# CVMI-Lab/DODA

Hardware: AMD Instinct MI355X
Metric: active-voxels/sec fwd+bwd SparseConv U-Net, ScanNet 2cm (higher is better)
Workload: dtype bf16; 1 GPU; cfgs/scannet SparseConv U-Net training step (voxel pooling + fwd + CE + bwd + SGD), 2 cm voxels, 4 scenes/GPU x ~150000 active voxels, random-init weights; global_batch=4, voxels_per_gpu=601279, points_per_gpu=781042, parallelism=dp1, n_classes=20, grad_sync=deferred multi-layer wgrad + bucketed all-reduce, collectives=none (single process), prefetch_gate=off, grad_exchange=no process group

## Files before the change

doda_amd/csrc/spconv_wgrad.hip:

```cpp
#include "wgrad_pairs.hpp"
#include <stdlib.h>
#include <string.h>
#include <mutex>
#include <vector>

typedef float f32x4 __attribute__((ext_vector_type(4)));
typedef short s16x4 __attribute__((ext_vector_type(4)));
typedef __bf16 bf16x8 __attribute__((ext_vector_type(8)));
typedef unsigned int u32x4 __attribute__((ext_vector_type(4)));

namespace {

constexpr int RT = 64;
constexpr int MAX_OGW = 7;
constexpr int PAD = 8;

struct F32 {
    typedef float elem;
    typedef f32x4 frag;
    typedef f32x4 vec;
    static constexpr int VEC = 4;
    static constexpr int KSTEPS = RT / 4;
    typedef float kfrag;
    template <int STRIDE>
    static __device__ __forceinline__ void frags(const elem *tile, int g, int i, int col0, kfrag (&out)[KSTEPS]) {
#pragma unroll
        for (int ks = 0; ks < KSTEPS; ++ks) out[ks] = tile[(ks * 4 + g) * STRIDE + col0 + i];
    }
    static __device__ __forceinline__ f32x4 mma(kfrag a, kfrag b, f32x4 c) {
        return __builtin_amdgcn_mfma_f32_16x16x4f32(a, b, c, 0, 0, 0);
    }
};

struct F32S : F32 {
    static constexpr int KSTEPS = RT / 16;
    struct kfrag { unsigned hi[2], lo[2]; };
    template <int STRIDE>
    static __device__ __forceinline__ void frags(const elem *tile, int g, int i, int col0, kfrag (&out)[KSTEPS]) {
        typedef __bf16 bf16x2 __attribute__((ext_vector_type(2)));
        typedef float f32x2 __attribute__((ext_vector_type(2)));
#pragma unroll
        for (int ks = 0; ks < KSTEPS; ++ks) {
            float v[4];
#pragma unroll
            for (int q = 0; q < 4; ++q) v[q] = tile[(ks * 16 + 4 * g + q) * STRIDE + col0 + i];
#pragma unroll
            for (int h = 0; h < 2; ++h) {
                const f32x2 a = {v[2 * h], v[2 * h + 1]};
                const unsigned hu = __builtin_bit_cast(unsigned, __builtin_convertvector(a, bf16x2));
                const f32x2 res = {a[0] - __uint_as_float(hu << 16), a[1] - __uint_as_float(hu & 0xffff0000u)};
                out[ks].hi[h] = hu;
                out[ks].lo[h] = __builtin_bit_cast(unsigned, __builtin_convertvector(res, bf16x2));
            }
        }
    }
    static __device__ __forceinline__ f32x4 mma(const kfrag &a, const kfrag &b, f32x4 c) {
        const u32x4 av = {a.hi[0], a.hi[1], a.lo[0], a.lo[1]};
        const u32x4 b1 = {b.hi[0], b.hi[1], b.hi[0], b.hi[1]}, b2 = {b.lo[0], b.lo[1], b.lo[0], b.lo[1]};
        c = __builtin_amdgcn_mfma_f32_16x16x32_bf16(__builtin_bit_cast(bf16x8, av), __builtin_bit_cast(bf16x8, b1), c, 0, 0, 0);
        return __builtin_amdgcn_mfma_f32_16x16x32_bf16(__builtin_bit_cast(bf16x8, av), __builtin_bit_cast(bf16x8, b2), c, 0, 0, 0);
    }
};

struct BF16 {
    typedef unsigned short elem;
    typedef s16x4 frag;
    typedef u32x4 vec;
    static constexpr int VEC = 8;
    static constexpr int KSTEPS = RT / 32;
    typedef bf16x8 kfrag;
    template <int STRIDE>
    static __device__ __forceinline__ void frags(const elem *tile, int g, int i, int col0, kfrag (&out)[KSTEPS]) {
        static_assert(KSTEPS == 2, "two k-steps of 32 rows");
        const unsigned addr = (unsigned)(uintptr_t)(tile + (8 * g + (i >> 2)) * STRIDE + col0 + 4 * (i & 3));
        s16x4 lo0, hi0, lo1, hi1;
        asm volatile("ds_read_b64_tr_b16 %0, %4\n\t"
                     "ds_read_b64_tr_b16 %1, %4 offset:%5\n\t"
                     "ds_read_b64_tr_b16 %2, %4 offset:%6\n\t"
                     "ds_read_b64_tr_b16 %3, %4 offset:%7\n\t"
                     "s_waitcnt lgkmcnt(0)"
                     : "=&v"(lo0), "=&v"(hi0), "=&v"(lo1), "=&v"(hi1)
                     : "v"(addr), "n"(4 * STRIDE * 2), "n"(32 * STRIDE * 2), "n"(36 * STRIDE * 2)
                     : "memory");
        typedef short s16x8 __attribute__((ext_vector_type(8)));
        const s16x8 k0 = __builtin_shufflevector(lo0, hi0, 0, 1, 2, 3, 4, 5, 6, 7);
        const s16x8 k1 = __builtin_shufflevector(lo1, hi1, 0, 1, 2, 3, 4, 5, 6, 7);
        out[0] = __builtin_bit_cast(bf16x8, k0);
        out[1] = __builtin_bit_cast(bf16x8, k1);
    }
    static __device__ __forceinline__ f32x4 mma(kfrag a, kfrag b, f32x4 c) {
        return __builtin_amdgcn_mfma_f32_16x16x32_bf16(a, b, c, 0, 0, 0);
    }
};

template <class T, int TA, int TB, int OGW, bool VOK>
__device__ __forceinline__ void wgrad_body(const typename T::elem *__restrict__ a, int ca,
                                           const typename T::elem *__restrict__ b, int cb,
                                           const int32_t *__restrict__ tbl, int ld, int K,
                                           int n_rows, int rows_per_chunk, int n_tag,
                                           int n_tbg, int n_og, float *__restrict__ partial, int item) {
    typedef typename T::elem elem;
    typedef typename T::frag frag;
    typedef typename T::kfrag kfrag;
    constexpr int SA = TA * 16 + PAD, SB = TB * 16 + PAD;
    __shared__ __attribute__((aligned(16))) elem b_tile[RT * SB];
    __shared__ __attribute__((aligned(16))) elem a_tile[4][RT * SA];

    const int lane = threadIdx.x & 63, wid = threadIdx.x >> 6;
    const int i = lane & 15, g = lane >> 4;
    const int n_grp = n_tag * n_tbg * n_og;
    const int chunk = item / n_grp;
    int grp = item % n_grp;
    const int tag = grp % n_tag; grp /= n_tag;
    const int tbg = grp % n_tbg;
    const int o_base = (grp / n_tbg) * (4 * OGW);
    const int ca0 = tag * TA * 16, cb0 = tbg * TB * 16;

    f32x4 acc[OGW][TA][TB];
#pragma unroll
    for (int oo = 0; oo < OGW; ++oo)
#pragma unroll
        for (int x_ = 0; x_ < TA; ++x_)
#pragma unroll
            for (int y_ = 0; y_ < TB; ++y_) acc[oo][x_][y_] = (f32x4){0.f, 0.f, 0.f, 0.f};

    const long long r_begin = (long long)chunk * rows_per_chunk;
    long long r_end = r_begin + rows_per_chunk;
    if (r_end > n_rows) r_end = n_rows;

    elem *my_a = a_tile[wid];

    typedef typename T::vec vec;
    constexpr int VEC = T::VEC, NVA = TA * 16 / VEC, NVB = TB * 16 / VEC;
    auto load_vec = [&](const elem *p, const elem *safe, int c, int cmax, bool ok) -> vec {
        const bool live = ok && c < cmax;
        if constexpr (VOK) {
            return *reinterpret_cast<const vec *>(live ? p : safe);
        } else {
            vec v = vec{};
            if (live) {
                elem tmp[VEC];
#pragma unroll
                for (int q = 0; q < VEC; ++q) tmp[q] = (c + q < cmax) ? p[q] : (elem)0;
                v = *reinterpret_cast<const vec *>(tmp);
            }
            return v;
        }
    };
    auto gather_row = [&](int idx, vec (&dst)[NVA]) {
#pragma unroll
        for (int f = 0; f < NVA; ++f) {
            const int c = ca0 + f * VEC;
            dst[f] = load_vec(a + (long long)(idx >= 0 ? idx : 0) * ca + c, a, c, ca, idx >= 0);
        }
    };

    constexpr int NDY = (RT * NVB + 255) / 256;
    vec dy_reg[NDY];
    int idx_n[OGW];
    auto load_dy = [&](long long r0) {
#pragma unroll
        for (int k = 0; k < NDY; ++k) {
            const int e = threadIdx.x + k * 256;
            const int r = e / NVB, f = e - r * NVB;
            const long long row = r0 + r;
            const int c = cb0 + f * VEC;
            dy_reg[k] = load_vec(b + (row < r_end ? row : 0) * cb + c, b, c, cb, e < RT * NVB && row < r_end);
        }
    };
    auto load_idx = [&](long long r0) {
#pragma unroll
        for (int oo = 0; oo < OGW; ++oo) {
            const int o = o_base + wid + 4 * oo;
            const long long row = r0 + lane;
            idx_n[oo] = tbl[(o < K && row < r_end) ? (long long)o * ld + row : 0];
        }
    };

    vec rows_cur[NVA], rows_nxt[NVA];
    if (r_begin < r_end) {
        load_dy(r_begin);
        load_idx(r_begin);
        gather_row((o_base + wid < K && r_begin + lane < r_end) ? idx_n[0] : -1, rows_cur);
    }
    for (long long r0 = r_begin; r0 < r_end; r0 += RT) {
        doda_sync();
#pragma unroll
        for (int k = 0; k < NDY; ++k) {
            const int e = threadIdx.x + k * 256;
            if (e < RT * NVB) {
                const int r = e / NVB, f = e - r * NVB;
                const bool live = r0 + r < r_end && cb0 + f * VEC < cb;
                *reinterpret_cast<vec *>(&b_tile[r * SB + f * VEC]) = (VOK && !live) ? vec{} : dy_reg[k];
            }
        }
        int idx[OGW];
#pragma unroll
        for (int oo = 0; oo < OGW; ++oo)
            idx[oo] = (o_base + wid + 4 * oo < K && r0 + lane < r_end) ? idx_n[oo] : -1;
        const bool more = r0 + RT < r_end;
        if (more) {
            load_dy(r0 + RT);
            load_idx(r0 + RT);
        }
        doda_sync();
        kfrag bf[TB][T::KSTEPS];
#pragma unroll
        for (int y_ = 0; y_ < TB; ++y_) T::template frags<SB>(b_tile, g, i, y_ * 16, bf[y_]);

#pragma unroll
        for (int oo = 0; oo < OGW; ++oo) {
            if (oo + 1 < OGW) gather_row(idx[oo + 1], rows_nxt);
            else if (more) gather_row((o_base + wid < K && r0 + RT + lane < r_end) ? idx_n[0] : -1, rows_nxt);
            if (__ballot(idx[oo] >= 0) != 0ull) {
#pragma unroll
                for (int f = 0; f < NVA; ++f) {
                    const bool live = idx[oo] >= 0 && ca0 + f * VEC < ca;
                    *reinterpret_cast<vec *>(&my_a[lane * SA + f * VEC]) = (VOK && !live) ? vec{} : rows_cur[f];
                }
                __builtin_amdgcn_wave_barrier();
#pragma unroll
                for (int x_ = 0; x_ < TA; ++x_) {
                    kfrag af[T::KSTEPS];
                    T::template frags<SA>(my_a, g, i, x_ * 16, af);
#pragma unroll
                    for (int ks = 0; ks < T::KSTEPS; ++ks)
#pragma unroll
                        for (int y_ = 0; y_ < TB; ++y_)
                            acc[oo][x_][y_] = T::mma(af[ks], bf[y_][ks], acc[oo][x_][y_]);
                }
                __builtin_amdgcn_wave_barrier();
            }
#pragma unroll
            for (int f = 0; f < NVA; ++f) rows_cur[f] = rows_nxt[f];
        }
    }

    float *out = partial + (long long)chunk * K * ca * cb;
#pragma unroll
    for (int oo = 0; oo < OGW; ++oo) {
        const int o = o_base + wid + 4 * oo;
        if (o < K) {
#pragma unroll
            for (int x_ = 0; x_ < TA; ++x_)
#pragma unroll
                for (int y_ = 0; y_ < TB; ++y_)
#pragma unroll
                    for (int r = 0; r < 4; ++r) {
                        const int ci = ca0 + x_ * 16 + 4 * g + r, co = cb0 + y_ * 16 + i;
                        if (ci < ca && co < cb)
                            out[((long long)o * ca + ci) * cb + co] = acc[oo][x_][y_][r];
                    }
        }
    }
}

struct WJob {
    const void *a, *b;
    const int32_t *tbl;
    float *out;
    int ca, cb, ld, K, n_rows, rows_per_chunk, n_tag, n_tbg, n_og, blk_end;
};
struct RJob {
    const float4 *partial;
    float4 *dw;
    long long n_quad;
    int R, blk_end, accumulate, pad;
};

template <class J>
__device__ __forceinline__ int find_job(const J *jobs, int n_jobs, int blk) {
    int lo = 0, hi = n_jobs - 1;
    while (lo < hi) {
        const int mid = (lo + hi) >> 1;
        if (blk < jobs[mid].blk_end) hi = mid; else lo = mid + 1;
    }
    return lo;
}

template <class T, int TA, int TB, int OGW, bool VOK>
__global__ __launch_bounds__(256) void wgrad_multi_kernel(const WJob *__restrict__ jobs, int n_jobs) {
    const int j = find_job(jobs, n_jobs, (int)blockIdx.x);
    const WJob d = jobs[j];
    const int first = j == 0 ? 0 : jobs[j - 1].blk_end;
    wgrad_body<T, TA, TB, OGW, VOK>((const typename T::elem *)d.a, d.ca, (const typename T::elem *)d.b, d.cb,
                                    d.tbl, d.ld, d.K, d.n_rows, d.rows_per_chunk, d.n_tag, d.n_tbg, d.n_og,
                                    d.out, (int)blockIdx.x - first);
}

__global__ __launch_bounds__(256) void wgrad_reduce_multi(const RJob *__restrict__ jobs, int n_jobs) {
    __shared__ float4 part[256];
    const int j = find_job(jobs, n_jobs, (int)blockIdx.x);
    const RJob d = jobs[j];
    const int first = j == 0 ? 0 : jobs[j - 1].blk_end;
    const int RL = d.pad, EL = 256 / RL;
    const int el = (int)threadIdx.x % EL, rl = (int)threadIdx.x / EL;
    const long long q = (long long)((int)blockIdx.x - first) * EL + el;
    float4 s = make_float4(0.f, 0.f, 0.f, 0.f);
    if (q < d.n_quad)
        for (int r = rl; r < d.R; r += RL) {
            const float4 v = d.partial[(long long)r * d.n_quad + q];
            s.x += v.x; s.y += v.y; s.z += v.z; s.w += v.w;
        }
    part[rl * EL + el] = s;
    doda_sync();
    if (rl == 0 && q < d.n_quad) {
        float4 t = part[el];
        for (int r = 1; r < RL; ++r) {
            const float4 v = part[r * EL + el];
            t.x += v.x; t.y += v.y; t.z += v.z; t.w += v.w;
        }
        if (d.accumulate) {
            const float4 old = d.dw[q];
            t.x += old.x; t.y += old.y; t.z += old.z; t.w += old.w;
        }
        d.dw[q] = t;
    }
}

__global__ __launch_bounds__(256) void wgrad_reduce(const float *__restrict__ partial, int R,
                                                    long long n_elem, float *__restrict__ dw,
                                                    int accumulate = 0) {
    __shared__ float part[16][17];
    const int el = threadIdx.x & 15, rl = threadIdx.x >> 4;
    const long long e = (long long)blockIdx.x * 16 + el;
    float s = 0.f;
    if (e < n_elem)
        for (int r = rl; r < R; r += 16) s += partial[(long long)r * n_elem + e];
    part[rl][el] = s;
    doda_sync();
    if (rl == 0 && e < n_elem) {
        float t = 0.f;
#pragma unroll
        for (int r = 0; r < 16; ++r) t += part[r][el];
        dw[e] = accumulate ? dw[e] + t : t;
    }
}


struct Plan {
    int TA, TB, OGW, n_og, n_tag, n_tbg, R, rows_per_chunk;
};
static const int MULTI_MIN_ROWS = getenv("DODA_WGRAD_MIN_ROWS") ? atoi(getenv("DODA_WGRAD_MIN_ROWS")) : 512;

Plan make_plan(int K, int ca, int cb, int n_rows, int elem_bytes, bool multi = false) {
    Plan p;
    const int ta = (ca + 15) / 16, tb = (cb + 15) / 16;
    p.TA = (ta % 2 == 0) ? 2 : 1;
    p.TB = (tb % 2 == 0) ? 2 : 1;
    static const bool no33 = getenv("DODA_WGRAD_NO33") && getenv("DODA_WGRAD_NO33")[0] == '1';
    if (ta == 3 && tb == 3 && elem_bytes == 2 && K > 8 && !no33) { p.TA = 3; p.TB = 3; }
    p.n_tag = ta / p.TA;
    p.n_tbg = tb / p.TB;
    p.OGW = (p.TA * p.TB == 4 || elem_bytes == 2) ? 4 : MAX_OGW;
    if (p.TA * p.TB == 9) p.OGW = 2;
    if (K <= 8) p.OGW = (p.TA * p.TB == 4) ? 2 : 2;
    p.n_og = div_up(K, 4 * p.OGW);
    const int gy = p.n_tag * p.n_tbg * p.n_og;
    const int rows = n_rows > 0 ? n_rows : 1;
    static const int t33 = getenv("DODA_WGRAD_T33") ? atoi(getenv("DODA_WGRAD_T33")) : 128;
    const int target = p.TA * p.TB == 9 ? t33 : (multi ? 512 : ((p.TA * p.TB == 4) ? 512 : 1024));
    int R = div_up(target, gy);
    const int max_r = multi ? (rows / MULTI_MIN_ROWS > 1 ? rows / MULTI_MIN_ROWS : 1) : div_up(rows, RT);
    if (R > max_r) R = max_r;
    if (R < 1) R = 1;
    p.rows_per_chunk = div_up(div_up(rows, R), RT) * RT;
    p.R = div_up(rows, p.rows_per_chunk);
    (void)K;
    return p;
}

struct JobPlan {
    Plan p;
    int esz, vok, key;
    int split;
    size_t ws_off;
    long long n_elem;
};

bool plan_job(const doda_wgrad_job &j, JobPlan *out) {
    if (j.ca <= 0 || j.cb <= 0 || j.K <= 0 || j.K > 4 * MAX_OGW || j.n_rows <= 0 || j.ld < j.n_rows || !j.a ||
        !j.b || !j.tbl || !j.dw || (j.elem_bytes != 2 && j.elem_bytes != 4))
        return false;
    out->esz = j.elem_bytes;
    out->vok = ((size_t)j.ca * j.elem_bytes % 16 == 0) && ((size_t)j.cb * j.elem_bytes % 16 == 0) &&
               ((uintptr_t)j.a % 16 == 0) && ((uintptr_t)j.b % 16 == 0);
    out->p = make_plan(j.K, j.ca, j.cb, j.n_rows, j.elem_bytes, true);
    {
        static const long long min_rows = [] { const char *e = getenv("DODA_F32_WGRAD_SPLIT_ROWS"); return e && *e ? atoll(e) : -1ll; }();
        out->split = (j.elem_bytes == 4 && min_rows >= 0 && (long long)j.n_rows >= min_rows) ? 1 : 0;
    }
    out->key = ((((j.elem_bytes * 4 + out->p.TA) * 4 + out->p.TB) * 8 + out->p.OGW) * 2 + out->vok) * 2 + out->split;
    out->n_elem = (long long)j.K * j.ca * j.cb;
    return true;
}

template <class T>
void launch_multi_variant(const Plan &p, int vok, int total_blocks, const WJob *jobs_dev, int n, hipStream_t s) {
    const dim3 grid(total_blocks), block(256);
#define GO(TA, TB, OG)                                                                             \
    do {                                                                                           \
        if (vok) hipLaunchKernelGGL((wgrad_multi_kernel<T, TA, TB, OG, true>), grid, block, 0, s, jobs_dev, n); \
        else hipLaunchKernelGGL((wgrad_multi_kernel<T, TA, TB, OG, false>), grid, block, 0, s, jobs_dev, n); \
    } while (0)
    if (p.OGW == 2) {
        if (p.TA == 3 && p.TB == 3) GO(3, 3, 2);
        else if (p.TA == 1 && p.TB == 1) GO(1, 1, 2);
        else if (p.TA == 2 && p.TB == 1) GO(2, 1, 2);
        else if (p.TA == 1 && p.TB == 2) GO(1, 2, 2);
        else GO(2, 2, 2);
    } else if (p.OGW == 4 && p.TA == 1 && p.TB == 1) GO(1, 1, 4);
    else if (p.OGW == 4 && p.TA == 2 && p.TB == 1) GO(2, 1, 4);
    else if (p.OGW == 4 && p.TA == 1 && p.TB == 2) GO(1, 2, 4);
    else if (p.TA == 1 && p.TB == 1) GO(1, 1, 7);
    else if (p.TA == 2 && p.TB == 1) GO(2, 1, 7);
    else if (p.TA == 1 && p.TB == 2) GO(1, 2, 7);
    else GO(2, 2, 4);
#undef GO
}

struct Staging {
    std::mutex mu;
    void *host = nullptr;
    size_t cap = 0;
    hipEvent_t ev = nullptr;
    int ev_dev = -1;
    bool pending = false;
};
Staging g_staging;
}

enum { J_SKIP = 0, J_ZERO = 1, J_DENSE = 2, J_PAIRS = 3, J_TILE = 4, J_WIDE = 5 };

static int wdma_min_rows() {
    static const int v = getenv("DODA_WDMA_MIN_ROWS") ? atoi(getenv("DODA_WDMA_MIN_ROWS")) : 32768;
    return v;
}

static int classify(const doda_wgrad_job &j) {
    if (j.n_rows == 0 && j.dw && j.K > 0 && j.ca > 0 && j.cb > 0)
        return (j.flags & DODA_WGRAD_ACCUMULATE) ? J_SKIP : J_ZERO;
    if (doda_wwide::eligible(j) && !doda_pairs::eligible(j)) return J_WIDE;
    if (j.tilebook && j.tbl && j.elem_bytes == 2 && j.ca % 16 == 0 && j.ca <= 64 && j.cb % 16 == 0 && j.cb <= 64 &&
        j.K == 27 && j.n_rows > 0 && j.a && j.b && j.dw &&
        j.n_a == j.n_rows && j.ld >= j.n_rows && (size_t)j.n_rows * 128 < 0x7ffffff0ull && (size_t)j.K * j.ld * 4 < 0xffffffffull &&
        !(((uintptr_t)j.a | (uintptr_t)j.b | (uintptr_t)j.tilebook) & 15) && doda_wdma::enabled() &&
        (j.n_rows >= wdma_min_rows() || !doda_pairs::eligible(j)))
        return J_TILE;
    static const bool no_pairs = getenv("DODA_WGRAD_NO_PAIRS") && getenv("DODA_WGRAD_NO_PAIRS")[0] == '1';
    if (doda_pairs::eligible(j) && (!no_pairs || !j.tbl)) return J_PAIRS;
    return J_DENSE;
}

static std::vector<int> wide_chunks(const doda_wgrad_job *jobs_h, const std::vector<int> &idx) {
    std::vector<int> rpc;
    for (int k : idx) rpc.push_back(make_plan(jobs_h[k].K, jobs_h[k].ca, jobs_h[k].cb, jobs_h[k].n_rows, 2, true).rows_per_chunk);
    return rpc;
}

static size_t tile_blocks(const doda_wgrad_job &j) { return (size_t)(j.ca / 16) * (j.cb / 16); }

static bool dense_needs_partial(const JobPlan &jp, const doda_wgrad_job &j) {
    return jp.p.R > 1 || (j.flags & DODA_WGRAD_ACCUMULATE);
}

extern "C" size_t doda_spconv_wgrad_multi_workspace_bytes(const doda_wgrad_job *jobs_h, int32_t n_jobs) {
    if (!jobs_h || n_jobs <= 0) return 0;
    size_t total = 0;
    std::vector<int> wide_jobs;
    for (int k = 0; k < n_jobs; ++k) {
        const int cls = classify(jobs_h[k]);
        if (cls == J_WIDE) { wide_jobs.push_back(k); continue; }
        if (cls == J_PAIRS) { total += doda_pairs::partial_bytes(jobs_h[k]); continue; }
        if (cls == J_TILE) { total += tile_blocks(jobs_h[k]) * align_up(doda_wdma::partial_bytes(jobs_h[k].n_rows), 256); continue; }
        if (cls != J_DENSE) continue;
        JobPlan jp;
        if (!plan_job(jobs_h[k], &jp)) continue;
        if (dense_needs_partial(jp, jobs_h[k])) total += align_up((size_t)jp.p.R * jp.n_elem * 4, 256);
    }
    const std::vector<int> rpc = wide_chunks(jobs_h, wide_jobs);
    total += doda_wwide::partial_bytes(jobs_h, wide_jobs.data(), rpc.data(), (int)wide_jobs.size());
    return total < 256 ? 256 : total;
}

extern "C" size_t doda_spconv_wgrad_multi_desc_bytes(int32_t n_jobs) {
    size_t per = sizeof(WJob) + sizeof(RJob) > doda_pairs::desc_bytes_per_job()
                     ? sizeof(WJob) + sizeof(RJob) : doda_pairs::desc_bytes_per_job();
    if (per < doda_wwide::desc_bytes_per_job()) per = doda_wwide::desc_bytes_per_job();
    return n_jobs <= 0 ? 0 : align_up((size_t)n_jobs * per + 256, 256);
}

extern "C" int doda_spconv_wgrad_multi(const doda_wgrad_job *jobs_h, int32_t n_jobs, void *ws, size_t ws_bytes,
                                       void *desc_dev, size_t desc_bytes, doda_stream_t stream) {
    if (!jobs_h || n_jobs <= 0 || !ws || !desc_dev) return DODA_ERR_INVALID;
    if (desc_bytes < doda_spconv_wgrad_multi_desc_bytes(n_jobs)) return DODA_ERR_WORKSPACE;
    hipStream_t s = as_stream(stream);
    std::vector<JobPlan> plans(n_jobs);
    std::vector<int> keys, cls(n_jobs), pair_jobs, tile_jobs, wide_jobs;
    size_t off = 0;
    for (int k = 0; k < n_jobs; ++k) {
        plans[k].key = -1;
        cls[k] = classify(jobs_h[k]);
        if (cls[k] == J_ZERO) {
            hipMemsetAsync(jobs_h[k].dw, 0, (size_t)jobs_h[k].K * jobs_h[k].ca * jobs_h[k].cb * 4, s);
            continue;
        }
        if (cls[k] == J_SKIP) continue;
        if (cls[k] == J_PAIRS) { pair_jobs.push_back(k); continue; }
        if (cls[k] == J_TILE) { tile_jobs.push_back(k); continue; }
        if (cls[k] == J_WIDE) { wide_jobs.push_back(k); continue; }
        if (!plan_job(jobs_h[k], &plans[k])) return DODA_ERR_INVALID;
        plans[k].ws_off = off;
        if (dense_needs_partial(plans[k], jobs_h[k])) off += align_up((size_t)plans[k].p.R * plans[k].n_elem * 4, 256);
        bool seen = false;
        for (int key : keys) seen |= key == plans[k].key;
        if (!seen) keys.push_back(plans[k].key);
    }
    doda_pairs::Prepared prep;
    if (!pair_jobs.empty()) {
        const int st = doda_pairs::prepare(jobs_h, pair_jobs.data(), (int)pair_jobs.size(), (char *)ws, &off, &prep);
        if (st != DODA_OK) return st;
    }
    {
        std::vector<char> done(tile_jobs.size(), 0);
        for (size_t q = 0; q < tile_jobs.size(); ++q) {
            if (done[q]) continue;
            const doda_wgrad_job &j0 = jobs_h[tile_jobs[q]];
            std::vector<doda_wdma::Block> blocks;
            for (size_t r = q; r < tile_jobs.size(); ++r) {
                const doda_wgrad_job &j = jobs_h[tile_jobs[r]];
                if (done[r] || j.tilebook != j0.tilebook || j.tbl != j0.tbl || j.n_rows != j0.n_rows || j.ld != j0.ld) continue;
                done[r] = 1;
                const int es = 2;
                for (int ci = 0; ci < j.ca; ci += 16)
                    for (int co = 0; co < j.cb; co += 16)
                        blocks.push_back(doda_wdma::Block{(const char *)j.a + ci * es, (const char *)j.b + co * es,
                                                          j.dw + (size_t)ci * j.cb + co, j.ca * es, j.cb * es, j.ca * j.cb, j.cb,
                                                          (j.flags & DODA_WGRAD_ACCUMULATE) ? 1 : 0});
            }
            const size_t bytes = blocks.size() * align_up(doda_wdma::partial_bytes(j0.n_rows), 256);
            if (ws_bytes < off + bytes) return DODA_ERR_WORKSPACE;
            const int st = doda_wdma::launch(blocks.data(), (int)blocks.size(), j0.tbl, j0.ld, j0.n_rows, j0.tilebook,
                                             (char *)ws + off, s);
            if (st != DODA_OK) return st;
            off += bytes;
        }
    }
    std::vector<unsigned char> wide_desc;
    int wide_wgs = 0, wide_red = 0;
    if (!wide_jobs.empty()) {
        const std::vector<int> rpc = wide_chunks(jobs_h, wide_jobs);
        const size_t bytes = doda_wwide::partial_bytes(jobs_h, wide_jobs.data(), rpc.data(), (int)wide_jobs.size());
        if (ws_bytes < off + bytes) return DODA_ERR_WORKSPACE;
        doda_wwide::prepare(jobs_h, wide_jobs.data(), rpc.data(), (int)wide_jobs.size(), (char *)ws + off, wide_desc, &wide_wgs,
                            &wide_red);
        off += bytes;
    }
    if (ws_bytes < off) return DODA_ERR_WORKSPACE;

    std::vector<WJob> wj;
    std::vector<RJob> rj;
    struct Group { int first, count, blocks, rep; };
    std::vector<Group> groups;
    for (int key : keys) {
        Group g{(int)wj.size(), 0, 0, -1};
        for (int k = 0; k < n_jobs; ++k) {
            if (cls[k] != J_DENSE || plans[k].key != key) continue;
            const doda_wgrad_job &j = jobs_h[k];
            const Plan &p = plans[k].p;
            if (g.rep < 0) g.rep = k;
            WJob d;
            d.a = j.a; d.b = j.b; d.tbl = j.tbl;
            d.out = dense_needs_partial(plans[k], j) ? (float *)((char *)ws + plans[k].ws_off) : j.dw;
            d.ca = j.ca; d.cb = j.cb; d.ld = j.ld; d.K = j.K; d.n_rows = j.n_rows;
            d.rows_per_chunk = p.rows_per_chunk; d.n_tag = p.n_tag; d.n_tbg = p.n_tbg; d.n_og = p.n_og;
            g.blocks += p.R * p.n_tag * p.n_tbg * p.n_og;
            d.blk_end = g.blocks;
            wj.push_back(d);
            ++g.count;
        }
        groups.push_back(g);
    }
    int r_blocks = 0;
    bool scalar_reduce = false;
    for (int k = 0; k < n_jobs; ++k) {
        if (cls[k] != J_DENSE || !dense_needs_partial(plans[k], jobs_h[k])) continue;
        if (plans[k].n_elem % 4 != 0 || (uintptr_t)jobs_h[k].dw % 16 != 0) { scalar_reduce = true; continue; }
        RJob d;
        d.partial = (const float4 *)((char *)ws + plans[k].ws_off);
        d.dw = (float4 *)jobs_h[k].dw;
        d.n_quad = plans[k].n_elem / 4;
        d.R = plans[k].p.R;
        d.accumulate = (jobs_h[k].flags & DODA_WGRAD_ACCUMULATE) ? 1 : 0;
        d.pad = 0;
        int rl = 1;
        while (rl < 16 && rl < d.R) rl *= 2;
        d.pad = rl;
        r_blocks += (int)div_up(d.n_quad, 256 / rl);
        d.blk_end = r_blocks;
        rj.push_back(d);
    }
    const size_t wbytes = wj.size() * sizeof(WJob), rbytes = rj.size() * sizeof(RJob);
    const size_t pair_off = align_up(wbytes + rbytes, 16), pbytes = prep.desc.size();
    const size_t wide_off = align_up(pair_off + pbytes, 16), wdbytes = wide_desc.size();
    const size_t total_desc = wide_off + wdbytes;
    if (total_desc > desc_bytes) return DODA_ERR_WORKSPACE;
    if (total_desc > 0) {
        std::lock_guard<std::mutex> lock(g_staging.mu);
        Staging &st = g_staging;
        if (st.pending) { hipEventSynchronize(st.ev); st.pending = false; }
        if (st.cap < total_desc) {
            if (st.host) hipHostFree(st.host);
            st.cap = align_up(total_desc, 4096) * 2;
            if (hipHostMalloc(&st.host, st.cap, hipHostMallocDefault) != hipSuccess) { st.host = nullptr; st.cap = 0; return DODA_ERR_NOMEM; }
        }
        int cur_dev = 0;
        hipGetDevice(&cur_dev);
        if (st.ev && st.ev_dev != cur_dev) { hipEventDestroy(st.ev); st.ev = nullptr; }
        if (!st.ev && hipEventCreateWithFlags(&st.ev, hipEventDisableTiming) != hipSuccess) return DODA_ERR_LAUNCH;
        st.ev_dev = cur_dev;
        if (wbytes) memcpy(st.host, wj.data(), wbytes);
        if (rbytes) memcpy((char *)st.host + wbytes, rj.data(), rbytes);
        if (pbytes) memcpy((char *)st.host + pair_off, prep.desc.data(), pbytes);
        if (wdbytes) memcpy((char *)st.host + wide_off, wide_desc.data(), wdbytes);
        if (hipMemcpyAsync(desc_dev, st.host, total_desc, hipMemcpyHostToDevice, s) != hipSuccess) return DODA_ERR_LAUNCH;
        hipEventRecord(st.ev, s);
        st.pending = true;
    }
    const WJob *wj_dev = (const WJob *)desc_dev;
    for (const Group &g : groups) {
        const JobPlan &jp = plans[g.rep];
        if (jp.esz == 4 && jp.split) launch_multi_variant<F32S>(jp.p, jp.vok, g.blocks, wj_dev + g.first, g.count, s);
        else if (jp.esz == 4) launch_multi_variant<F32>(jp.p, jp.vok, g.blocks, wj_dev + g.first, g.count, s);
        else launch_multi_variant<BF16>(jp.p, jp.vok, g.blocks, wj_dev + g.first, g.count, s);
    }
    int st = doda_check_launch();
    if (st != DODA_OK) return st;
    if (!pair_jobs.empty()) {
        st = doda_pairs::launch(prep, (const char *)desc_dev + pair_off, s);
        if (st != DODA_OK) return st;
    }
    if (!wide_jobs.empty()) {
        st = doda_wwide::launch((const char *)desc_dev + wide_off, (int)wide_jobs.size(), wide_wgs, wide_red, s);
        if (st != DODA_OK) return st;
    }
    if (!rj.empty()) {
        hipLaunchKernelGGL(wgrad_reduce_multi, dim3(r_blocks), dim3(256), 0, s,
                           (const RJob *)((const char *)desc_dev + wbytes), (int)rj.size());
        st = doda_check_launch();
        if (st != DODA_OK) return st;
    }
    if (scalar_reduce)
        for (int k = 0; k < n_jobs; ++k) {
            if (cls[k] != J_DENSE || !dense_needs_partial(plans[k], jobs_h[k])) continue;
            if (plans[k].n_elem % 4 == 0 && (uintptr_t)jobs_h[k].dw % 16 == 0) continue;
            hipLaunchKernelGGL(wgrad_reduce, dim3(div_up(plans[k].n_elem, 16)), dim3(256), 0, s,
                               (const float *)((char *)ws + plans[k].ws_off), plans[k].p.R, plans[k].n_elem,
                               jobs_h[k].dw, (jobs_h[k].flags & DODA_WGRAD_ACCUMULATE) ? 1 : 0);
        }
    return doda_check_launch();
}
```

doda_amd/csrc/wgrad_pairs.hpp:

```cpp
#pragma once
#include "common.hpp"
#include <vector>

namespace doda_pairs {

bool eligible(const doda_wgrad_job &j);

size_t partial_bytes(const doda_wgrad_job &j);

struct Prepared {
    std::vector<unsigned char> desc;
    struct Group { int ta, tb, first, count, blocks; };
    std::vector<Group> groups;
    size_t reduce_off = 0;
    int n_reduce = 0, reduce_blocks = 0;
};

int prepare(const doda_wgrad_job *jobs, const int *which, int n, char *ws_base, size_t *ws_off, Prepared *out);

int launch(const Prepared &p, const void *desc_dev, hipStream_t s);

size_t desc_bytes_per_job();

}

namespace doda_wdma {
bool enabled();
void set_enabled(bool on);
int max_jobs();
size_t partial_bytes(int n_rows);
struct Block { const void *x, *dy; float *dw; int x_stride, dy_stride, ldo, ldc, accumulate; };
int launch(const Block *blocks, int n_blocks, const int32_t *tbl, int ld, int n_rows, const void *tilebook, void *part,
           hipStream_t s);
}

namespace doda_wwide {
bool eligible(const doda_wgrad_job &j);
size_t partial_bytes(const doda_wgrad_job *jobs, const int *idx, const int *rows_per_chunk, int n);
size_t desc_bytes_per_job();
void prepare(const doda_wgrad_job *jobs, const int *idx, const int *rows_per_chunk, int n, void *part,
             std::vector<unsigned char> &desc, int *wgs, int *red_blocks);
int launch(const void *desc_dev, int n, int wgs, int red_blocks, hipStream_t s);
}
```

Measured before the change: 136.7 million voxels/s.

## Add one-source wgrad kernel sharing dy tile across up to eight offsets

Adds a new weight-gradient path for jobs with at most eight kernel offsets that are not pair-eligible. Each workgroup stages one dy tile in LDS and reuses it for up to eight offsets, one wave per offset, gathering each wave's input rows through the index table. It uses bf16 MFMA with software double buffering, and its partial results feed the existing reduce kernel. The aim is to cut redundant dy loads and launch overhead compared with the generic dense path. In exchange it adds LDS pressure and leaves waves idle when K is below eight.

```diff
diff --git a/doda_amd/csrc/spconv_wgrad.hip b/doda_amd/csrc/spconv_wgrad.hip
--- a/doda_amd/csrc/spconv_wgrad.hip
+++ b/doda_amd/csrc/spconv_wgrad.hip
@@ -430,7 +430,7 @@
 Staging g_staging;
 }
 
-enum { J_SKIP = 0, J_ZERO = 1, J_DENSE = 2, J_PAIRS = 3, J_TILE = 4, J_WIDE = 5 };
+enum { J_SKIP = 0, J_ZERO = 1, J_DENSE = 2, J_PAIRS = 3, J_TILE = 4, J_WIDE = 5, J_ONE = 6 };
 
 static int wdma_min_rows() {
     static const int v = getenv("DODA_WDMA_MIN_ROWS") ? atoi(getenv("DODA_WDMA_MIN_ROWS")) : 32768;
@@ -447,6 +447,7 @@
         !(((uintptr_t)j.a | (uintptr_t)j.b | (uintptr_t)j.tilebook) & 15) && doda_wdma::enabled() &&
         (j.n_rows >= wdma_min_rows() || !doda_pairs::eligible(j)))
         return J_TILE;
+    if (doda_wone::eligible(j) && !doda_pairs::eligible(j)) return J_ONE;
     static const bool no_pairs = getenv("DODA_WGRAD_NO_PAIRS") && getenv("DODA_WGRAD_NO_PAIRS")[0] == '1';
     if (doda_pairs::eligible(j) && (!no_pairs || !j.tbl)) return J_PAIRS;
     return J_DENSE;
@@ -473,7 +474,7 @@
         if (cls == J_WIDE) { wide_jobs.push_back(k); continue; }
         if (cls == J_PAIRS) { total += doda_pairs::partial_bytes(jobs_h[k]); continue; }
         if (cls == J_TILE) { total += tile_blocks(jobs_h[k]) * align_up(doda_wdma::partial_bytes(jobs_h[k].n_rows), 256); continue; }
-        if (cls != J_DENSE) continue;
+        if (cls != J_DENSE && cls != J_ONE) continue;
         JobPlan jp;
         if (!plan_job(jobs_h[k], &jp)) continue;
         if (dense_needs_partial(jp, jobs_h[k])) total += align_up((size_t)jp.p.R * jp.n_elem * 4, 256);
@@ -487,6 +488,7 @@
     size_t per = sizeof(WJob) + sizeof(RJob) > doda_pairs::desc_bytes_per_job()
                      ? sizeof(WJob) + sizeof(RJob) : doda_pairs::desc_bytes_per_job();
     if (per < doda_wwide::desc_bytes_per_job()) per = doda_wwide::desc_bytes_per_job();
+    if (per < doda_wone::desc_bytes_per_job() + sizeof(RJob)) per = doda_wone::desc_bytes_per_job() + sizeof(RJob);
     return n_jobs <= 0 ? 0 : align_up((size_t)n_jobs * per + 256, 256);
 }
 
@@ -496,7 +498,7 @@
     if (desc_bytes < doda_spconv_wgrad_multi_desc_bytes(n_jobs)) return DODA_ERR_WORKSPACE;
     hipStream_t s = as_stream(stream);
     std::vector<JobPlan> plans(n_jobs);
-    std::vector<int> keys, cls(n_jobs), pair_jobs, tile_jobs, wide_jobs;
+    std::vector<int> keys, cls(n_jobs), pair_jobs, tile_jobs, wide_jobs, one_jobs;
     size_t off = 0;
     for (int k = 0; k < n_jobs; ++k) {
         plans[k].key = -1;
@@ -512,6 +514,7 @@
         if (!plan_job(jobs_h[k], &plans[k])) return DODA_ERR_INVALID;
         plans[k].ws_off = off;
         if (dense_needs_partial(plans[k], jobs_h[k])) off += align_up((size_t)plans[k].p.R * plans[k].n_elem * 4, 256);
+        if (cls[k] == J_ONE) { one_jobs.push_back(k); continue; }
         bool seen = false;
         for (int key : keys) seen |= key == plans[k].key;
         if (!seen) keys.push_back(plans[k].key);
@@ -558,6 +561,18 @@
     }
     if (ws_bytes < off) return DODA_ERR_WORKSPACE;
 
+    std::vector<unsigned char> one_desc;
+    int one_wgs = 0;
+    if (!one_jobs.empty()) {
+        std::vector<int> rpc;
+        std::vector<float *> outs;
+        for (int k : one_jobs) {
+            rpc.push_back(plans[k].p.rows_per_chunk);
+            outs.push_back(dense_needs_partial(plans[k], jobs_h[k]) ? (float *)((char *)ws + plans[k].ws_off) : jobs_h[k].dw);
+        }
+        doda_wone::prepare(jobs_h, one_jobs.data(), rpc.data(), outs.data(), (int)one_jobs.size(), one_desc, &one_wgs);
+    }
+
     std::vector<WJob> wj;
     std::vector<RJob> rj;
     struct Group { int first, count, blocks, rep; };
@@ -584,7 +599,7 @@
     int r_blocks = 0;
     bool scalar_reduce = false;
     for (int k = 0; k < n_jobs; ++k) {
-        if (cls[k] != J_DENSE || !dense_needs_partial(plans[k], jobs_h[k])) continue;
+        if ((cls[k] != J_DENSE && cls[k] != J_ONE) || !dense_needs_partial(plans[k], jobs_h[k])) continue;
         if (plans[k].n_elem % 4 != 0 || (uintptr_t)jobs_h[k].dw % 16 != 0) { scalar_reduce = true; continue; }
         RJob d;
         d.partial = (const float4 *)((char *)ws + plans[k].ws_off);
@@ -603,7 +618,8 @@
     const size_t wbytes = wj.size() * sizeof(WJob), rbytes = rj.size() * sizeof(RJob);
     const size_t pair_off = align_up(wbytes + rbytes, 16), pbytes = prep.desc.size();
     const size_t wide_off = align_up(pair_off + pbytes, 16), wdbytes = wide_desc.size();
-    const size_t total_desc = wide_off + wdbytes;
+    const size_t one_off = align_up(wide_off + wdbytes, 16), odbytes = one_desc.size();
+    const size_t total_desc = one_off + odbytes;
     if (total_desc > desc_bytes) return DODA_ERR_WORKSPACE;
     if (total_desc > 0) {
         std::lock_guard<std::mutex> lock(g_staging.mu);
@@ -623,6 +639,7 @@
         if (rbytes) memcpy((char *)st.host + wbytes, rj.data(), rbytes);
         if (pbytes) memcpy((char *)st.host + pair_off, prep.desc.data(), pbytes);
         if (wdbytes) memcpy((char *)st.host + wide_off, wide_desc.data(), wdbytes);
+        if (odbytes) memcpy((char *)st.host + one_off, one_desc.data(), odbytes);
         if (hipMemcpyAsync(desc_dev, st.host, total_desc, hipMemcpyHostToDevice, s) != hipSuccess) return DODA_ERR_LAUNCH;
         hipEventRecord(st.ev, s);
         st.pending = true;
@@ -644,6 +661,10 @@
         st = doda_wwide::launch((const char *)desc_dev + wide_off, (int)wide_jobs.size(), wide_wgs, wide_red, s);
         if (st != DODA_OK) return st;
     }
+    if (!one_jobs.empty()) {
+        st = doda_wone::launch((const char *)desc_dev + one_off, (int)one_jobs.size(), one_wgs, s);
+        if (st != DODA_OK) return st;
+    }
     if (!rj.empty()) {
         hipLaunchKernelGGL(wgrad_reduce_multi, dim3(r_blocks), dim3(256), 0, s,
                            (const RJob *)((const char *)desc_dev + wbytes), (int)rj.size());
@@ -652,7 +673,7 @@
     }
     if (scalar_reduce)
         for (int k = 0; k < n_jobs; ++k) {
-            if (cls[k] != J_DENSE || !dense_needs_partial(plans[k], jobs_h[k])) continue;
+            if ((cls[k] != J_DENSE && cls[k] != J_ONE) || !dense_needs_partial(plans[k], jobs_h[k])) continue;
             if (plans[k].n_elem % 4 == 0 && (uintptr_t)jobs_h[k].dw % 16 == 0) continue;
             hipLaunchKernelGGL(wgrad_reduce, dim3(div_up(plans[k].n_elem, 16)), dim3(256), 0, s,
                                (const float *)((char *)ws + plans[k].ws_off), plans[k].p.R, plans[k].n_elem,
diff --git a/doda_amd/csrc/spconv_wone.hip b/doda_amd/csrc/spconv_wone.hip
--- /dev/null
+++ b/doda_amd/csrc/spconv_wone.hip
@@ -0,0 +1,219 @@
+#include "wgrad_pairs.hpp"
+#include <stdlib.h>
+#include <string.h>
+
+namespace {
+
+typedef float f32x4o __attribute__((ext_vector_type(4)));
+typedef short s16x4o __attribute__((ext_vector_type(4)));
+typedef __bf16 bf16x8o __attribute__((ext_vector_type(8)));
+typedef unsigned int u32x4o __attribute__((ext_vector_type(4)));
+
+constexpr int WO_WAVES = 8;
+constexpr int WO_RT = 64;
+constexpr int WO_PAD = 8;
+constexpr int WO_MAX_T = 3;
+constexpr int wo_lds_elems(int ta, int tb) { return 2 * WO_RT * (16 * tb + WO_PAD) + WO_WAVES * WO_RT * (16 * ta + WO_PAD); }
+constexpr int WO_SMEM = wo_lds_elems(WO_MAX_T, WO_MAX_T) * 2;
+
+struct WoJob {
+    const unsigned short *a, *b;
+    const int32_t *tbl;
+    float *out;
+    int ca, cb, ld, K, n_rows, rpc, ta, tb, n_sa, n_sb, wg_end, pad;
+};
+
+__device__ __forceinline__ int wo_find(const WoJob *jobs, int n, int blk) {
+    int lo = 0, hi = n - 1;
+    while (lo < hi) {
+        const int mid = (lo + hi) >> 1;
+        if (blk < jobs[mid].wg_end) hi = mid; else lo = mid + 1;
+    }
+    return lo;
+}
+
+__device__ __forceinline__ u32x4o wo_ldg(const unsigned short *p) {
+    return *(const __attribute__((address_space(1))) u32x4o *)(uintptr_t)p;
+}
+__device__ __forceinline__ int wo_ldg_i(const int32_t *p) {
+    return *(const __attribute__((address_space(1))) int *)(uintptr_t)p;
+}
+__device__ __forceinline__ s16x4o wo_tr(const unsigned short *p) {
+    return __builtin_amdgcn_ds_read_tr16_b64_v4i16((__attribute__((address_space(3))) s16x4o *)(uintptr_t)p);
+}
+template <int STRIDE>
+__device__ __forceinline__ void wo_frags(const unsigned short *tile, int g, int i, int col0, bf16x8o (&out)[2]) {
+    const unsigned short *p = tile + (8 * g + (i >> 2)) * STRIDE + col0 + 4 * (i & 3);
+    const s16x4o lo0 = wo_tr(p), hi0 = wo_tr(p + 4 * STRIDE), lo1 = wo_tr(p + 32 * STRIDE), hi1 = wo_tr(p + 36 * STRIDE);
+    out[0] = __builtin_bit_cast(bf16x8o, __builtin_shufflevector(lo0, hi0, 0, 1, 2, 3, 4, 5, 6, 7));
+    out[1] = __builtin_bit_cast(bf16x8o, __builtin_shufflevector(lo1, hi1, 0, 1, 2, 3, 4, 5, 6, 7));
+}
+
+template <int TA, int TB>
+__device__ void wo_body(const WoJob &d, int local, unsigned short *smem) {
+    constexpr int SA = TA * 16 + WO_PAD, SB = TB * 16 + WO_PAD;
+    constexpr int NVA = TA * 2, NVB = TB * 2;
+    static_assert(WO_RT * NVB <= WO_WAVES * 64, "one dy vector per thread and step");
+    const int tid = threadIdx.x, lane = tid & 63, wid = __builtin_amdgcn_readfirstlane(tid >> 6);
+    const int i = lane & 15, g = lane >> 4;
+    const int n_sl = d.n_sa * d.n_sb;
+    const int chunk = local / n_sl, sl = local - chunk * n_sl;
+    const int sa = sl / d.n_sb, sb = sl - sa * d.n_sb;
+    const int ca0 = sa * TA * 16, cb0 = sb * TB * 16;
+    const int r_begin = chunk * d.rpc;
+    const int r_end = min(d.n_rows, r_begin + d.rpc);
+    const bool has_o = wid < d.K;
+    unsigned short *b_tile = smem;
+    unsigned short *my_a = smem + 2 * WO_RT * SB + wid * WO_RT * SA;
+    unsigned short *dump = smem + WO_SMEM / 2;
+
+    f32x4o acc[TA][TB];
+#pragma unroll
+    for (int x = 0; x < TA; ++x)
+#pragma unroll
+        for (int y = 0; y < TB; ++y) acc[x][y] = (f32x4o){0.f, 0.f, 0.f, 0.f};
+
+    const int32_t *tb_o = d.tbl + (size_t)(has_o ? wid : 0) * d.ld;
+    const bool dy_thr = tid < WO_RT * NVB;
+    const int dy_r = dy_thr ? tid / NVB : 0, dy_f = dy_thr ? tid - (tid / NVB) * NVB : 0;
+    auto load_idx = [&](int r0) -> int {
+        const int row = r0 + lane;
+        return wo_ldg_i(tb_o + (row < r_end ? row : r_begin));
+    };
+    auto load_rows = [&](int r0, int idx, u32x4o (&v)[NVA], bool &live) {
+        live = has_o && idx >= 0 && r0 + lane < r_end;
+        const unsigned short *p = d.a + (size_t)(idx >= 0 ? idx : 0) * d.ca + ca0;
+#pragma unroll
+        for (int f = 0; f < NVA; ++f) v[f] = wo_ldg(p + f * 8);
+    };
+    auto load_dy = [&](int r0, u32x4o &v, bool &live) {
+        const int row = r0 + dy_r;
+        live = dy_thr && row < r_end;
+        v = wo_ldg(d.b + (size_t)(row < r_end ? row : r_begin) * d.cb + cb0 + dy_f * 8);
+    };
+    const u32x4o zero = {0u, 0u, 0u, 0u};
+
+    auto step = [&](int r0, int par, u32x4o (&rows)[NVA], bool &rows_live, u32x4o &dy, bool &dy_live, int &idx_use,
+                    int &idx_load) {
+        idx_load = load_idx(r0 + 3 * WO_RT);
+        __builtin_amdgcn_sched_barrier(0);
+        unsigned short *bt = b_tile + par * WO_RT * SB;
+        *reinterpret_cast<u32x4o *>(dy_thr ? bt + dy_r * SB + dy_f * 8 : dump) = dy_live ? dy : zero;
+#pragma unroll
+        for (int f = 0; f < NVA; ++f) *reinterpret_cast<u32x4o *>(my_a + lane * SA + f * 8) = rows_live ? rows[f] : zero;
+        __builtin_amdgcn_sched_barrier(0);
+        load_rows(r0 + 2 * WO_RT, idx_use, rows, rows_live);
+        load_dy(r0 + 2 * WO_RT, dy, dy_live);
+        __builtin_amdgcn_sched_barrier(0);
+        doda_sync();
+        if (has_o) {
+            bf16x8o bf[TB][2];
+#pragma unroll
+            for (int y = 0; y < TB; ++y) wo_frags<SB>(bt, g, i, y * 16, bf[y]);
+#pragma unroll
+            for (int x = 0; x < TA; ++x) {
+                bf16x8o af[2];
+                wo_frags<SA>(my_a, g, i, x * 16, af);
+#pragma unroll
+                for (int ks = 0; ks < 2; ++ks)
+#pragma unroll
+                    for (int y = 0; y < TB; ++y)
+                        acc[x][y] = __builtin_amdgcn_mfma_f32_16x16x32_bf16(af[ks], bf[y][ks], acc[x][y], 0, 0, 0);
+            }
+        }
+        __builtin_amdgcn_sched_barrier(0);
+    };
+
+    u32x4o rows_a[NVA], rows_b[NVA], dy_a, dy_b;
+    bool la, lb, dla, dlb;
+    int idx_u, idx_v;
+    {
+        const int i0 = load_idx(r_begin), i1 = load_idx(r_begin + WO_RT);
+        idx_v = 0;
+        load_rows(r_begin, i0, rows_a, la);
+        load_dy(r_begin, dy_a, dla);
+        __builtin_amdgcn_sched_barrier(0);
+        idx_u = load_idx(r_begin + 2 * WO_RT);
+        __builtin_amdgcn_sched_barrier(0);
+        load_rows(r_begin + WO_RT, i1, rows_b, lb);
+        load_dy(r_begin + WO_RT, dy_b, dlb);
+        __builtin_amdgcn_sched_barrier(0);
+    }
+#pragma unroll 1
+    for (int r0 = r_begin; r0 < r_end; r0 += 2 * WO_RT) {
+        step(r0, 0, rows_a, la, dy_a, dla, idx_u, idx_v);
+        step(r0 + WO_RT, 1, rows_b, lb, dy_b, dlb, idx_v, idx_u);
+    }
+
+    if (has_o) {
+        float *out = d.out + ((size_t)chunk * d.K + wid) * d.ca * d.cb;
+#pragma unroll
+        for (int x = 0; x < TA; ++x)
+#pragma unroll
+            for (int y = 0; y < TB; ++y)
+#pragma unroll
+                for (int r = 0; r < 4; ++r)
+                    out[(size_t)(ca0 + x * 16 + 4 * g + r) * d.cb + cb0 + y * 16 + i] = acc[x][y][r];
+    }
+}
+
+#define WO_SHAPES(X) X(1, 1) X(1, 2) X(1, 3) X(2, 1) X(2, 2) X(2, 3) X(3, 1) X(3, 2) X(3, 3)
+
+__global__ __launch_bounds__(WO_WAVES * 64) void wgrad_one(const WoJob *__restrict__ jobs, int n_jobs) {
+    __shared__ __attribute__((aligned(16))) unsigned short smem[WO_SMEM / 2 + 8];
+    const int j = wo_find(jobs, n_jobs, (int)blockIdx.x);
+    const WoJob d = jobs[j];
+    const int local = (int)blockIdx.x - (j == 0 ? 0 : jobs[j - 1].wg_end);
+#define WO_CASE(A, B) if (d.ta == A && d.tb == B) { wo_body<A, B>(d, local, smem); return; }
+    WO_SHAPES(WO_CASE)
+#undef WO_CASE
+}
+
+int wo_side(int c) {
+    const int n = c / 16;
+    int t = WO_MAX_T;
+    while (t > 1 && n % t) --t;
+    return t;
+}
+
+}
+
+namespace doda_wone {
+
+bool eligible(const doda_wgrad_job &j) {
+    static const bool on = !(getenv("DODA_WGRAD_ONESRC") && getenv("DODA_WGRAD_ONESRC")[0] == '0');
+    return on && j.tbl && j.elem_bytes == 2 && j.K >= 1 && j.K <= WO_WAVES && j.n_rows > 0 && j.a && j.b && j.dw &&
+           j.ca > 0 && j.cb > 0 && j.ca % 16 == 0 && j.cb % 16 == 0 && j.ca <= 224 && j.cb <= 224 && j.ld >= j.n_rows &&
+           !(((uintptr_t)j.a | (uintptr_t)j.b | (uintptr_t)j.dw) & 15) &&
+           (size_t)j.n_rows * 448 < 0x7ffffff0ull && (size_t)j.K * j.ld * 4 < 0xffffffffull;
+}
+
+size_t desc_bytes_per_job() { return sizeof(WoJob); }
+
+void prepare(const doda_wgrad_job *jobs, const int *idx, const int *rows_per_chunk, float *const *out, int n,
+             std::vector<unsigned char> &desc, int *wgs) {
+    std::vector<WoJob> v;
+    int total = 0;
+    for (int k = 0; k < n; ++k) {
+        const doda_wgrad_job &j = jobs[idx[k]];
+        WoJob d;
+        memset(&d, 0, sizeof(d));
+        d.a = (const unsigned short *)j.a; d.b = (const unsigned short *)j.b; d.tbl = j.tbl; d.out = out[k];
+        d.ca = j.ca; d.cb = j.cb; d.ld = j.ld; d.K = j.K; d.n_rows = j.n_rows; d.rpc = rows_per_chunk[k];
+        d.ta = wo_side(j.ca); d.tb = wo_side(j.cb);
+        d.n_sa = j.ca / (16 * d.ta); d.n_sb = j.cb / (16 * d.tb);
+        total += div_up(j.n_rows, d.rpc) * d.n_sa * d.n_sb;
+        d.wg_end = total;
+        v.push_back(d);
+    }
+    desc.resize(v.size() * sizeof(WoJob));
+    if (!v.empty()) memcpy(desc.data(), v.data(), desc.size());
+    *wgs = total;
+}
+
+int launch(const void *desc_dev, int n, int wgs, hipStream_t s) {
+    hipLaunchKernelGGL(wgrad_one, dim3(wgs), dim3(WO_WAVES * 64), 0, s, (const WoJob *)desc_dev, n);
+    return doda_check_launch();
+}
+
+}
diff --git a/doda_amd/csrc/wgrad_pairs.hpp b/doda_amd/csrc/wgrad_pairs.hpp
--- a/doda_amd/csrc/wgrad_pairs.hpp
+++ b/doda_amd/csrc/wgrad_pairs.hpp
@@ -42,3 +42,11 @@
              std::vector<unsigned char> &desc, int *wgs, int *red_blocks);
 int launch(const void *desc_dev, int n, int wgs, int red_blocks, hipStream_t s);
 }
+
+namespace doda_wone {
+bool eligible(const doda_wgrad_job &j);
+size_t desc_bytes_per_job();
+void prepare(const doda_wgrad_job *jobs, const int *idx, const int *rows_per_chunk, float *const *out, int n,
+             std::vector<unsigned char> &desc, int *wgs);
+int launch(const void *desc_dev, int n, int wgs, hipStream_t s);
+}
```

Result: no change. 137.7 million voxels/s (median of 3 runs) (+0.7%).
